# wangxb29/PPST

Hardware: AMD Instinct MI355X
Metric: 512x512 portrait swaps/sec/GPU (higher is better)
Workload: dtype bf16x3 (fp32 split into hi+lo bf16, 3 MFMA passes, fp32 accumulate); 1 GPU; simple_swapping 512x512 batch=8 per GPU, generator+encoders forward only (BASELINE configs[1]); image_parallel=1 batch per rank, no data-path collective

## Files before the change

include/ppst_hip.h:

```cpp
#ifndef PPST_HIP_H
#define PPST_HIP_H

#include <stddef.h>
#include <stdint.h>

#ifdef __cplusplus
extern "C" {
#endif

#define PPST_OK 0
#define PPST_EINVAL (-1)
#define PPST_EUNSUPPORTED (-2)
#define PPST_ENULL (-3)

enum { PPST_F32 = 0, PPST_F16 = 1, PPST_BF16 = 2, PPST_F64 = 3  };

enum { PPST_PAD_ZERO = 0, PPST_PAD_REFLECT = 1, PPST_PAD_REPLICATE = 2 };

enum { PPST_ACT_NONE = 0, PPST_ACT_LRELU = 1 , PPST_ACT_PRELU = 2 };

#define PPST_ABI_VERSION 3
int ppst_version(void);

#define PPST_ST_F32 0
// ... 61 lines not shown
  int32_t cout, cin, nblocks;
} ppst_upscale_job;
int ppst_pack_job_blocks(int64_t total);
int ppst_conv_pack_batch(const void* jobs, int njobs, int total_blocks, void* stream);
int ppst_upscale_weight_batch(const void* jobs, int njobs, int total_blocks, void* stream);

int ppst_upscale_weight(const void* w, void* out, int cout, int cin, float scale, void* stream);
int ppst_dgrad_s2d_stack_weight(const void* w, void* out, int cout, int cin, void* stream);
int ppst_depth_to_space_st(const void* x, void* y, int B, int th, int tw, int oh, int ow, int C, int st, void* stream);

#define PPST_KSPLIT_SCRATCH_BYTES ((size_t)256 * 512 * 128 * 4)
#define PPST_KSPLIT_FLAG_WORDS 4096

typedef struct ppst_conv_args {
  const void* x;
  const void* wpack;
  const void* steps;
  void* y;
  const void* bias;
  const void* noise;
  const void* prelu;
  void* stats;
  const void* residual;
  float noise_weight;
  float out_scale;
  int32_t B, in_h, in_w, in_ld;
  int32_t out_h, out_w, out_ld, cout;
  int32_t nsteps, n_groups;
  int32_t pad_mode;
  int32_t in_off_y, in_off_x;
  int32_t out_sy, out_sx;
  int32_t act;
  int32_t precision;
  int32_t res_ld;
  int32_t tile_h, tile_w;
  int32_t halo;
  int32_t bn;
  const void* in_scale_shift;
  const void* in_prelu;
  int32_t in_c, in_act;
  int32_t flop_steps;
  int32_t tile_rows;
  int32_t a_slots;
  int32_t early_a;
  int32_t variant;
  int32_t reserved0;
  int32_t dual_b;
  int32_t io_st;
  int32_t k64;
  const void* in_res;
  int32_t in_res_ld;
  int32_t ksplit;
  const int32_t* ksplit_starts;
  void* ksplit_scratch;
  unsigned* ksplit_flags;
  uint32_t ksplit_epoch;
} ppst_conv_args;

int ppst_conv2d_mfma(const ppst_conv_args* a, void* stream);
int64_t ppst_conv_pack_wino_bytes(int cout, int cin);
int ppst_conv_pack_wino(const void* w, int64_t sn, int64_t sc, int64_t sy, int64_t sx, float scale, int cout, int cin,
                        void* out, void* stream);
int ppst_conv2d_f32(const ppst_conv_args* a, const void* w, int64_t sn, int64_t sc, int64_t sy, int64_t sx, float wscale,
                    const int32_t* src_c, const int32_t* src_ky, const int32_t* src_kx, void* stream);
int ppst_conv_tiles(int tile_h, int tile_w, int tile_rows);

int ppst_conv1x1_small_cin(const void* x, const void* w, const void* bias, void* y,
                           int64_t npix, int cin, int in_ld, int cout, float wscale,
                           int act, void* stream);
int ppst_conv1x1_small_cin_st(const void* x, const void* w, const void* bias, void* y,
                              int64_t npix, int cin, int in_ld, int cout, float wscale,
                              int act, int y_st , void* stream);
int ppst_conv1x1_small_cin_nchw_st(const void* x, const void* w, const void* bias, void* y, int B, int64_t hw, int cin, int cout,
                                   float wscale, int act, int y_st, void* stream);
int ppst_conv1x1_small_cout(const void* x, const void* w, const void* bias, void* y,
                            int64_t npix, int cin, int cout, float wscale, void* stream);
int ppst_conv1x1_small_cout_st(const void* x, const void* w, const void* bias, void* y,
                               int64_t npix, int cin, int cout, float wscale, int x_st , void* stream);
int ppst_conv1x1_small_cout_ld_st(const void* x, const void* w, const void* bias, void* y, int64_t npix, int cin, int in_ld, int cout,
                                  float wscale, int x_st, void* stream);
int ppst_torgb_linear_st(const void* x, const void* scale_shift, const void* proj, float out_scale, const void* w, const void* bias,
                        void* y, void* partial, int* n_partials, int B, int H, int W, int cin, float wscale, int x_st, void* stream);
int ppst_rgb_affine_nchw(const void* y, const void* scale_shift, void* out, int B, int64_t hw, void* stream);

int ppst_in_stats(const void* x, void* partial, int B, int H, int W, int C, int ld,
                  int rep_pad, int* n_partials, void* stream);
int ppst_in_finalize(const void* partial, int n_partials, const void* style,
                     int style_ld ,
                     const void* post_bias ,
                     void* scale_shift , int B, int C, double count,
                     float eps, void* stream);
int ppst_affine_act(const void* x, const void* scale_shift, const void* res,
                    const void* res_scale_shift , void* y,
                    int B, int64_t hw, int C, int x_ld, int res_ld, int y_ld,
                    int act , const void* prelu,
                    float out_scale,
                    int res_up2_w ,
                    void* stream);
int ppst_affine_act_st(const void* x, const void* scale_shift, const void* res, const void* res_scale_shift, void* y,
                       int B, int64_t hw, int C, int x_ld, int res_ld, int y_ld, int act, const void* prelu,
                       float out_scale, int res_up2_w, int x_st, int y_st, void* stream);
int ppst_affine_act_stats(const void* x, const void* scale_shift, const void* res,
                          const void* res_scale_shift, void* y, void* partial,
                          int B, int H, int W, int C, int x_ld, int res_ld, int y_ld,
                          int act, const void* prelu, float out_scale, int rep_pad,
                          int res_up2 , void* stream);
int ppst_upsample_nearest2(const void* x, void* y, int B, int H, int W, int C, void* stream);
int ppst_upsample_nearest2_st(const void* x, void* y, int B, int H, int W, int C, int st, void* stream);

int64_t ppst_gap_gmp_ws(int B, int64_t hw, int C);
int ppst_gap_gmp(const void* x, const void* mask, void* out, void* ws, int B, int H, int W,
                 int C, int ld, void* stream);
int ppst_gap_gmp_st(const void* x, const void* mask, void* out, void* ws, int B, int H, int W,
                    int C, int ld, int x_st, void* stream);
#define PPST_GROUP_MAX 32
typedef struct {
  const void* x;
  const void* mask;
  void* out;
  int32_t H, W, C, ld;
} ppst_gap_gmp_level;
int64_t ppst_gap_gmp_multi_level_ws(const ppst_gap_gmp_level* levels, int n, int B);
int ppst_gap_gmp_multi_level(const ppst_gap_gmp_level* levels, int n, int B, void* ws, int x_st, void* stream);
int ppst_avgpool(const void* x, void* y, int B, int H, int W, int C, int x_ld, int f,
                 int y_ld, void* stream);
int ppst_bilinear(const void* x, void* y, int B, int H, int W, int C, int x_ld,
                  int OH, int OW, int y_ld, void* stream);
int ppst_head_tail(const void* x, const void* scale_shift, const void* prelu, void* feat, void* feat1,
                   int B, int H, int W, int C, int x_ld, int feat_ld, int feat1_ld, int P, int D, int act,
                   void* stream);
int ppst_maxpool2(const void* x, void* y, int B, int H, int W, int C, void* stream);

int ppst_linear(const void* x, const void* w, const void* bias, void* y,
                int B, int K, int N, float wscale, float bscale, int relu_in, int act,
                void* stream);
int ppst_l2norm_rows(const void* x, void* y, int B, int K, float eps, int mode, void* stream);
int ppst_lerp(const void* a, const void* b, void* y, int64_t n, float r, void* stream);
typedef struct {
  const void* x; const void* w; const void* bias ; void* y;
  int32_t B, K, N;
  float wscale, bscale;
  int32_t relu_in, act;
} ppst_linear_problem;
typedef struct { const void* x; void* y; int32_t B, K; float eps; int32_t mode; } ppst_l2norm_problem;
typedef struct { const void* a; const void* b; void* y; int64_t n; float r; } ppst_lerp_problem;
int ppst_linear_grouped(const ppst_linear_problem* problems, int n, void* stream);
int ppst_l2norm_rows_grouped(const ppst_l2norm_problem* problems, int n, void* stream);
int ppst_lerp_grouped(const ppst_lerp_problem* problems, int n, void* stream);
int ppst_spatial_modulation(const void* x, const void* scale, const void* bias, void* y,
                            int B, int64_t hw, int C, void* stream);
int ppst_spatial_modulation_st(const void* x, const void* scale, const void* bias, void* y,
                               int B, int64_t hw, int C, int y_st , void* stream);

int ppst_rselfcorr(const void* fea, void* out, int B, int H, int W, int C, int out_ld,
                   void* stream);
int ppst_corr_prep(const void* fea, void* out, int B, int P, int C, int ncenter, void* stream);
int ppst_unfold_rows(const void* x, void* out, int B, int H, int W, int C, int k, void* stream);
int ppst_unfold_rows_bwd(const void* g, void* dx, int B, int H, int W, int C, int k, void* stream);
int ppst_gemm_nt_f32(const void* A, const void* Bm, void* C, int batch, int M, int N, int K,
                     float alpha, void* stream);
int ppst_gemm_nn_f32(const void* A, const void* Bm, void* C, int batch, int M, int N, int K,
                     int ldb, int ldc, void* stream);
int ppst_gemm_nt_split(const void* A, const void* Bm, void* C, int batch, int M, int N, int K,
                       float alpha, int passes, void* stream);
int ppst_gemm_nn_split(const void* A, const void* Bm, void* C, int batch, int M, int N, int K,
                       int ldb, int ldc, int passes, void* stream);
// ... 263 lines not shown
```

ppst_amd/_lib.py:

```python
import ctypes
import os

import torch

HERE = os.path.dirname(os.path.abspath(__file__))
LIB_PATH = os.environ.get("PPST_HIP_LIB") or os.path.join(HERE, "libppst_hip.so")

if not os.path.exists(LIB_PATH):
    raise ImportError(
        "ppst_amd: %s is missing -- build it with `python -m ppst_amd.build` "
        "(hipcc --offload-arch=gfx950). There is no CPU fallback." % LIB_PATH)

lib = ctypes.CDLL(LIB_PATH)

vp, i32, i64, f32, f64 = ctypes.c_void_p, ctypes.c_int, ctypes.c_int64, ctypes.c_float, ctypes.c_double


class PackJob(ctypes.Structure):
    _fields_ = [("w", vp), ("sn", i64), ("sc", i64), ("sy", i64), ("sx", i64), ("src_c", vp), ("src_ky", vp), ("src_kx", vp),
                ("out", vp), ("total", i64), ("block0", i64), ("scale", f32), ("cout", i32), ("bn", i32), ("nsteps", i32),
                ("n_groups", i32), ("x3", i32), ("f16", i32), ("nblocks", i32), ("dual", i32)]


class UpscaleJob(ctypes.Structure):
# ... 7 lines not shown

class L2normProblem(ctypes.Structure):
    _fields_ = [("x", vp), ("y", vp), ("B", i32), ("K", i32), ("eps", f32), ("mode", i32)]


class LerpProblem(ctypes.Structure):
    _fields_ = [("a", vp), ("b", vp), ("y", vp), ("n", i64), ("r", f32)]


class GapGmpLevel(ctypes.Structure):
    _fields_ = [("x", vp), ("mask", vp), ("out", vp), ("H", i32), ("W", i32), ("C", i32), ("ld", i32)]


class JpegDecImage(ctypes.Structure):
    _u8 = ctypes.c_uint8
    _fields_ = [("H", i32), ("W", i32), ("ncomp", i32), ("ss", i32), ("hs", i32 * 3), ("vs", i32 * 3), ("dri", i32),
                ("scan_off", i32), ("scan_len", i32), ("qt", _u8 * 64 * 3), ("dc_tab", _u8 * 3), ("ac_tab", _u8 * 3), ("pad_", _u8 * 2),
                ("bits", _u8 * 16 * 4), ("vals", _u8 * 256 * 4), ("file_off", i64), ("out_off", i64), ("mirror", i32), ("expand_grey", i32)]


class PngSpan(ctypes.Structure):
    _fields_ = [("type", ctypes.c_uint32), ("off", i32), ("len", i32), ("crc", ctypes.c_uint32), ("idat", i32)]


class PngDecImage(ctypes.Structure):
    _fields_ = [("H", i32), ("W", i32), ("colour", i32), ("channels", i32), ("nspans", i32), ("first_idat", i32), ("nidat", i32),
                ("idat_bytes", i32), ("file_len", i64), ("file_off", i64), ("out_off", i64), ("span_off", i64),
                ("mirror", i32), ("expand_grey", i32), ("drop_alpha", i32), ("pad_", i32)]


GROUP_MAX = 32


class ConvArgs(ctypes.Structure):
    _fields_ = [
        ("x", vp), ("wpack", vp), ("steps", vp), ("y", vp), ("bias", vp), ("noise", vp),
        ("prelu", vp), ("stats", vp), ("residual", vp),
        ("noise_weight", f32), ("out_scale", f32),
        ("B", i32), ("in_h", i32), ("in_w", i32), ("in_ld", i32),
        ("out_h", i32), ("out_w", i32), ("out_ld", i32), ("cout", i32),
        ("nsteps", i32), ("n_groups", i32), ("pad_mode", i32),
        ("in_off_y", i32), ("in_off_x", i32), ("out_sy", i32), ("out_sx", i32),
        ("act", i32), ("precision", i32), ("res_ld", i32), ("tile_h", i32), ("tile_w", i32),
        ("halo", i32), ("bn", i32), ("in_scale_shift", vp), ("in_prelu", vp), ("in_c", i32), ("in_act", i32),
        ("flop_steps", i32), ("tile_rows", i32), ("a_slots", i32), ("early_a", i32), ("variant", i32), ("reserved0", i32), ("dual_b", i32), ("io_st", i32), ("k64", i32),
        ("in_res", vp), ("in_res_ld", i32), ("ksplit", i32), ("ksplit_starts", vp),
        ("ksplit_scratch", vp), ("ksplit_flags", vp), ("ksplit_epoch", ctypes.c_uint32),
    ]


_SIGS = {
    "ppst_version": (i32, []),
    "ppst_guided_filter_tune": (i32, [i32, i32]),
    "ppst_upfirdn2d": (i32, [vp, vp, vp] + [i32] * 14 + [i32, vp]),
    "ppst_blur_nhwc": (i32, [vp, vp, vp] + [i32] * 10 + [vp, i32, vp]),
    "ppst_blur_nhwc_st": (i32, [vp, vp, vp] + [i32] * 10 + [vp, i32, i32, vp]),
    "ppst_fused_bias_act": (i32, [vp, vp, vp, vp, i64, i32, i32, i32, i32, f32, f32, i32, vp]),
    "ppst_nchw_to_nhwc": (i32, [vp, vp, i32, i32, i32, i32, vp]),
    "ppst_nhwc_to_nchw": (i32, [vp, vp, i32, i32, i32, i32, vp]),
    "ppst_conv_pack": (i32, [vp, i64, i64, i64, i64, f32, i32, i32, vp, vp, vp, i32, i32, i32, vp, vp]),
    "ppst_conv_pack_k64": (i32, [vp, i64, i64, i64, i64, f32, i32, i32, vp, vp, vp, i32, i32, i32, i32, vp, vp]),
    "ppst_conv_pack_up9_bytes": (i64, [i32, i32]),
    "ppst_conv_pack_up9": (i32, [vp, i64, i64, i64, i64, f32, i32, i32, vp, vp]),
    "ppst_conv_pack_wino_bytes": (i64, [i32, i32]),
    "ppst_conv_pack_wino": (i32, [vp, i64, i64, i64, i64, f32, i32, i32, vp, vp]),
    "ppst_conv_pack_dual": (i32, [vp, i64, i64, i64, i64, f32, i32, vp, vp, vp, i32, i32, i32, vp, vp]),
    "ppst_upscale_weight": (i32, [vp, vp, i32, i32, f32, vp]),
    "ppst_dgrad_s2d_stack_weight": (i32, [vp, vp, i32, i32, vp]),
    "ppst_depth_to_space_st": (i32, [vp, vp, i32, i32, i32, i32, i32, i32, i32, vp]),
    "ppst_pack_job_blocks": (i32, [i64]),
    "ppst_conv_pack_batch": (i32, [vp, i32, i32, vp]),
    "ppst_upscale_weight_batch": (i32, [vp, i32, i32, vp]),
    "ppst_conv2d_mfma": (i32, [ctypes.POINTER(ConvArgs), vp]),
    "ppst_conv2d_f32": (i32, [ctypes.POINTER(ConvArgs), vp, i64, i64, i64, i64, f32, vp, vp, vp, vp]),
    "ppst_conv_tiles": (i32, [i32, i32, i32]),
    "ppst_conv1x1_small_cin": (i32, [vp, vp, vp, vp, i64, i32, i32, i32, f32, i32, vp]),
    "ppst_conv1x1_small_cin_st": (i32, [vp, vp, vp, vp, i64, i32, i32, i32, f32, i32, i32, vp]),
    "ppst_conv1x1_small_cout": (i32, [vp, vp, vp, vp, i64, i32, i32, f32, vp]),
    "ppst_conv1x1_small_cin_nchw_st": (i32, [vp, vp, vp, vp, i32, i64, i32, i32, f32, i32, i32, vp]),
    "ppst_conv1x1_small_cout_st": (i32, [vp, vp, vp, vp, i64, i32, i32, f32, i32, vp]),
    "ppst_conv1x1_small_cout_ld_st": (i32, [vp, vp, vp, vp, i64, i32, i32, i32, f32, i32, vp]),
    "ppst_torgb_linear_st": (i32, [vp, vp, vp, f32, vp, vp, vp, vp, ctypes.POINTER(i32), i32, i32, i32, i32, f32, i32, vp]),
    "ppst_rgb_affine_nchw": (i32, [vp, vp, vp, i32, i64, vp]),
    "ppst_in_stats": (i32, [vp, vp, i32, i32, i32, i32, i32, i32, ctypes.POINTER(i32), vp]),
    "ppst_in_finalize": (i32, [vp, i32, vp, i32, vp, vp, i32, i32, f64, f32, vp]),
    "ppst_affine_act": (i32, [vp, vp, vp, vp, vp, i32, i64, i32, i32, i32, i32, i32, vp, f32, i32, vp]),
    "ppst_affine_act_st": (i32, [vp, vp, vp, vp, vp, i32, i64, i32, i32, i32, i32, i32, vp, f32, i32, i32, i32, vp]),
    "ppst_affine_act_stats": (i32, [vp, vp, vp, vp, vp, vp, i32, i32, i32, i32, i32, i32, i32, i32, vp, f32, i32, i32, vp]),
    "ppst_upsample_nearest2": (i32, [vp, vp, i32, i32, i32, i32, vp]),
    "ppst_upsample_nearest2_st": (i32, [vp, vp, i32, i32, i32, i32, i32, vp]),
    "ppst_gap_gmp_ws": (i64, [i32, i64, i32]),
    "ppst_gap_gmp": (i32, [vp, vp, vp, vp, i32, i32, i32, i32, i32, vp]),
    "ppst_gap_gmp_st": (i32, [vp, vp, vp, vp, i32, i32, i32, i32, i32, i32, vp]),
    "ppst_avgpool": (i32, [vp, vp, i32, i32, i32, i32, i32, i32, i32, vp]),
    "ppst_bilinear": (i32, [vp, vp, i32, i32, i32, i32, i32, i32, i32, i32, vp]),
    "ppst_head_tail": (i32, [vp, vp, vp, vp, vp] + [i32] * 10 + [vp]),
    "ppst_maxpool2": (i32, [vp, vp, i32, i32, i32, i32, vp]),
    "ppst_linear": (i32, [vp, vp, vp, vp, i32, i32, i32, f32, f32, i32, i32, vp]),
    "ppst_l2norm_rows": (i32, [vp, vp, i32, i32, f32, i32, vp]),
    "ppst_lerp": (i32, [vp, vp, vp, i64, f32, vp]),
    "ppst_linear_grouped": (i32, [vp, i32, vp]),
    "ppst_l2norm_rows_grouped": (i32, [vp, i32, vp]),
    "ppst_lerp_grouped": (i32, [vp, i32, vp]),
    "ppst_gap_gmp_multi_level_ws": (i64, [vp, i32, i32]),
    "ppst_gap_gmp_multi_level": (i32, [vp, i32, i32, vp, i32, vp]),
    "ppst_spatial_modulation": (i32, [vp, vp, vp, vp, i32, i64, i32, vp]),
    "ppst_spatial_modulation_st": (i32, [vp, vp, vp, vp, i32, i64, i32, i32, vp]),
    "ppst_rselfcorr": (i32, [vp, vp, i32, i32, i32, i32, i32, vp]),
    "ppst_corr_prep": (i32, [vp, vp, i32, i32, i32, i32, vp]),
    "ppst_gemm_nt_f32": (i32, [vp, vp, vp, i32, i32, i32, i32, f32, vp]),
    "ppst_gemm_nn_f32": (i32, [vp, vp, vp, i32, i32, i32, i32, i32, i32, vp]),
    "ppst_unfold_rows": (i32, [vp, vp, i32, i32, i32, i32, i32, vp]),
    "ppst_unfold_rows_bwd": (i32, [vp, vp, i32, i32, i32, i32, i32, vp]),
    "ppst_gemm_nt_split": (i32, [vp, vp, vp, i32, i32, i32, i32, f32, i32, vp]),
    "ppst_gemm_nn_split": (i32, [vp, vp, vp, i32, i32, i32, i32, i32, i32, i32, vp]),
    "ppst_softmax_rows": (i32, [vp, i64, i32, f32, vp]),
    "ppst_unfold_patches": (i32, [vp, vp, i32, i32, i32, i32, i32, vp]),
    "ppst_fold_patches": (i32, [vp, vp, i32, i32, i32, i32, i32, vp]),
    "ppst_tensor2im_u8": (i32, [vp, vp, i32, i32, i32, i32, vp]),
    "ppst_resample_u8": (i32, [vp, vp, i32, i32, i32, i32, i32, i32, vp, vp, i32, vp]),
    "ppst_u8_to_tensor": (i32, [vp, vp, i32, i32, i32, i32, f32, f32, vp]),
    "ppst_resample_f32": (i32, [vp, vp, i32, i32, i32, i32, i32, vp, vp, i32, vp, vp, i32, i32, f32, f32, vp]),
    "ppst_png_bound": (i64, [i32, i32, i32]),
    "ppst_png_ws": (i64, [i32, i32, i32, i32]),
    "ppst_png_encode": (i32, [vp, vp, vp, i32, i32, i32, i32, vp, vp]),
    "ppst_jpeg_bound": (i64, [i32, i32, i32, i32]),
    "ppst_jpeg_ws": (i64, [i32, i32, i32, i32, i32]),
    "ppst_jpeg_header": (i64, [i32, i32, i32, i32, i32, vp, i64]),
    "ppst_jpeg_encode": (i32, [vp, vp, vp, i32, i32, i32, i32, i32, i32, vp, vp]),
    "ppst_jpeg_parse": (i32, [vp, i64, ctypes.POINTER(JpegDecImage)]),
    "ppst_jpeg_decode_ws": (i64, [ctypes.POINTER(JpegDecImage), i32, i32]),
    "ppst_jpeg_decode": (i32, [vp, i64, ctypes.POINTER(JpegDecImage), vp, vp, i64, vp, i32, i32, vp, vp]),
    "ppst_png_parse": (i32, [vp, i64, ctypes.POINTER(PngDecImage), ctypes.POINTER(PngSpan), i32]),
    "ppst_png_decode_ws": (i64, [ctypes.POINTER(PngDecImage), i32, i32]),
    "ppst_png_decode": (i32, [vp, i64, ctypes.POINTER(PngDecImage), vp, vp, vp, i64, vp, i32, i32, vp, vp]),
    "ppst_lpips_pack_floats": (i64, []),
    "ppst_lpips_pack": (i32, [vp, vp, vp, vp, vp, vp, vp]),
    "ppst_lpips_dims": (i32, [i32, i32, ctypes.POINTER(i32)]),
    "ppst_lpips_ws": (i64, [i32, i32, i32]),
    "ppst_lpips_trunk": (i32, [vp, vp, ctypes.POINTER(i64), i32, vp, ctypes.POINTER(i64), i32, i32, i32, vp, vp]),
    "ppst_lpips_feature": (i32, [vp, i32, i32, i32, i32, vp, vp]),
    "ppst_lpips_tail": (i32, [vp, vp, i32, i32, i32, vp, vp]),
    "ppst_lpips_bwd_ws": (i64, [i32, i32, i32, i32]),
    "ppst_lpips_backward": (i32, [vp, vp, vp, i32, i32, i32, i32, vp, vp, vp, vp]),
    "ppst_ssim_ws": (i64, [i32, i32, i32, i32]),
    "ppst_ssim_forward": (i32, [vp, ctypes.POINTER(i64), vp, ctypes.POINTER(i64), i32, i32, i32, i32, i32, f32, vp, vp, vp, vp, vp]),
    "ppst_ssim_backward": (i32, [vp, ctypes.POINTER(i64), vp, ctypes.POINTER(i64), vp, i32, i32, i32, i32, f32, vp, vp]),
    "ppst_pool2x2": (i32, [vp, ctypes.POINTER(i64), i32, i32, i32, i32, i32, vp, vp]),
    "ppst_msssim_combine": (i32, [vp, i32, i32, vp, vp]),
    "ppst_sqerr_ws": (i64, [i32, i32, i32, i32]),
    "ppst_sqerr": (i32, [vp, ctypes.POINTER(i64), vp, ctypes.POINTER(i64), i32, i32, i32, i32, i32, f32, vp, vp, vp]),
    "ppst_colour_stats_ws": (i64, [i32, i32, i32]),
    "ppst_colour_stats": (i32, [vp, i64, i64, i64, vp, i64, i64, i32, i32, i32, i32, ctypes.POINTER(ctypes.c_int16), i32, vp, vp, vp, vp, vp, vp]),
    "ppst_hist_w1": (i32, [vp, i32, vp, i32, vp, i32, i32, i32, vp, vp]),
    "ppst_guided_filter_ws": (i64, [i32, i32, i32]),
    "ppst_guided_filter": (i32, [vp, vp, vp, vp, i32, i32, i32, i32, f32, vp, vp]),
    "ppst_guided_filter_coeffs": (i32, [vp, vp, vp, i32, i32, i32, i32, f32, vp, vp]),
    "ppst_guided_filter_apply": (i32, [vp, i32, i32, vp, vp, vp, i32, i32, i32, vp]),
    "ppst_guided_filter_paste": (i32, [vp, i32, vp, vp, i32, i32, i32, vp, vp, i32, vp]),
    "ppst_guided_filter_paste_matte": (i32, [vp, vp, i32, vp, vp, i32, i32, i32, vp, vp, i32, vp]),
    "ppst_label_matte": (i32, [vp, i32, i32, i32, ctypes.c_uint32, i32, i32, vp, vp, vp]),
    "ppst_extract_similarity": (i32, [vp, i32, i32, i32, vp, vp, i32, vp, vp]),
    "ppst_smooth_local_affine_ws": (i64, [i32, i32, i32]),
    "ppst_smooth_local_affine": (i32, [vp, vp, vp, vp, vp, i32, i32, i32, i32, i32, f32, f32, vp]),
    "ppst_conv_wgrad_f32": (i32, [vp, vp, vp, vp, vp] + [i32] * 11 + [vp]),
    "ppst_conv_wgrad_tr2": (i32, [vp, vp, vp, vp, vp, vp, i32, i32, i32, i32, i32, i32, i32, i32, i32, i32, i32, i32, i32, i32, i32, vp]),
# ... 95 lines not shown
```

ppst_amd/build.py:

```python
import os
import subprocess
import sys
from concurrent.futures import ThreadPoolExecutor

HERE = os.path.dirname(os.path.abspath(__file__))
CSRC = os.path.join(HERE, "csrc")
OBJ = os.path.join(HERE, "csrc", "_obj")
LIB = os.path.join(HERE, "libppst_hip.so")
SOURCES = ["upfirdn2d.hip", "fused_bias_act.hip", "elementwise.hip", "linear.hip", "conv_mfma.hip", "conv_mfma2.hip", "conv1x1.hip", "conv_wino.hip", "conv_f32.hip",
           "corr.hip", "guided_filter.hip", "train.hip", "train_g.hip", "imageio.hip", "smooth_filter.hip", "png.hip", "jpeg.hip", "jpeg_parse.hip", "jpeg_decode.hip", "png_parse.hip", "png_decode.hip", "lpips.hip", "ssim.hip", "colour_stats.hip", "matte.hip"]
FLAGS = ["--offload-arch=gfx950", "-O3", "-fPIC", "-std=c++17", "-Wno-unused-result"]
FILE_FLAGS = {"conv_wino.hip": ["-fno-slp-vectorize"]}


def _hipcc():
    for c in (os.environ.get("HIPCC"), "/opt/rocm/bin/hipcc", "hipcc"):
        if c and (os.path.isabs(c) and os.path.exists(c) or not os.path.isabs(c)):
            return c
    return "hipcc"


HEADERS = [os.path.join(CSRC, "common.h"), os.path.join(CSRC, "conv_common.h"), os.path.join(CSRC, "rscl_common.h"), os.path.join(CSRC, "png_common.h"),
           os.path.join(CSRC, "codec_common.h"), os.path.join(CSRC, "jpeg_common.h"), os.path.join(CSRC, "parse_reader.h"), os.path.join(CSRC, "sim_xf.h"),
           os.path.join(HERE, "..", "include", "ppst_hip.h")]


def _stale(target, deps):
    return not os.path.exists(target) or any(os.path.getmtime(d) > os.path.getmtime(target) for d in deps)


def needs_build():
    return (_stale(LIB, [os.path.join(CSRC, s) for s in SOURCES] + HEADERS) or
            any(_stale(os.path.join(OBJ, s.replace(".hip", ".o")), [os.path.join(CSRC, s)]) for s in SOURCES if os.path.isdir(OBJ)))


def build(force=False, verbose=True):
    if not force and not needs_build():
        return LIB
    os.makedirs(OBJ, exist_ok=True)
    hipcc = _hipcc()

    def cc(src):
        obj = os.path.join(OBJ, src.replace(".hip", ".o"))
        if not force and not _stale(obj, [os.path.join(CSRC, src)] + HEADERS):
            return obj
        cmd = [hipcc] + FLAGS + FILE_FLAGS.get(src, []) + ["-c", os.path.join(CSRC, src), "-o", obj]
        r = subprocess.run(cmd, capture_output=True, text=True)
        if r.returncode != 0:
            raise RuntimeError("hipcc failed for %s:\n%s" % (src, r.stderr))
        return obj

    order = sorted(SOURCES, key=lambda f: 0 if f.startswith("conv") else 1)
    with ThreadPoolExecutor(max_workers=8) as ex:
        objs = dict(zip(order, ex.map(cc, order)))
    cmd = [hipcc, "--offload-arch=gfx950", "-shared", "-fPIC", "-o", LIB] + [objs[s_] for s_ in SOURCES]
    r = subprocess.run(cmd, capture_output=True, text=True)
    if r.returncode != 0:
        raise RuntimeError("link failed:\n%s" % r.stderr)
    if verbose:
        print("built", LIB)
    return LIB


if __name__ == "__main__":
    build(force="--force" in sys.argv)
```

ppst_amd/networks/base_network.py:

```python
import math

import torch
from torch import nn

from .. import ops, weights

SQRT2 = math.sqrt(2.0)
INV_SQRT2 = 1.0 / SQRT2


class _Node(nn.Module):
    """parameter container (no behaviour)."""


def to_nhwc(x):
    if x.dim() != 4:
        raise RuntimeError("expected a 4-D NCHW tensor")
    v = x.permute(0, 2, 3, 1)
    if v.is_contiguous():
        ops._chk(v, "input")
        return v
    return ops.nchw_to_nhwc(x)


# ... 29 lines not shown

    def p(self, name):
        t = self._flat.get(name)
        if t is None:
            node = self
            parts = name.split(".")
            for part in parts[:-1]:
                node = node._modules[part]
            t = node._parameters.get(parts[-1])
            if t is None:
                t = node._buffers[parts[-1]]
            self._flat[name] = t
        return t

    def _apply(self, fn, *a, **k):
        self._flat.clear()
        self._cache.clear()
        return super()._apply(fn, *a, **k)

    def load_state_dict(self, *a, **k):
        self._flat.clear()
        self._cache.clear()
        return super().load_state_dict(*a, **k)

    def cached(self, key, params, build):
        ver = tuple((id(t), t._version, t.data_ptr()) for t in params) + (ops.PRECISION["value"],)
        hit = self._cache.get(key)
        if hit is not None and hit[0] == ver:
            return hit[1]
        val = build()
        self._cache[key] = (ver, val)
        return val

    def plan(self, wname, kind="conv", scale=1.0):
        w = self.p(wname)
        return self.cached(("plan", wname, kind), [w], lambda: ops.ConvPlan(w, kind=kind, scale=scale))

    def refresh_plans(self):
        plans, keep = [], {}
        for key, (ver, val) in self._cache.items():
            if isinstance(key, tuple) and key and key[0] == "plan" and isinstance(val, ops.ConvPlan) and val.precision != 2 \
                    and val.wparam.data_ptr() == self.p(key[1]).data_ptr():
                plans.append(val)
                keep[key] = (ver, val)
        self._cache.clear()
        if not plans:
            return
        sig = tuple((id(pl), tuple(sorted(map(str, pl._packs)))) for pl in plans)
        hit = self.__dict__.get("_repack")
        if hit is not None and hit[0] == sig:
            ops.run_repack(hit[1])
        else:
            self.__dict__["_repack"] = (sig, ops.repack_plans(plans), plans)
        self._cache.update(keep)

    def print_architecture(self, verbose=False):
        n = sum(p.numel() for p in self.parameters())
        print("[Network %s] Total number of parameters : %.3f M" % (type(self).__name__, n / 1e6))

    def from_rgb(self, x, p, out_dtype=torch.float32):
        w = self.p(p + "Conv.weight")
        return ops.conv1x1_small_cin(x, w, self.p(p + "Act.bias"), 1.0 / math.sqrt(w.shape[1]), ops.ACT_LRELU, out_dtype=out_dtype)

    def from_rgb_image(self, img, p, out_dtype=torch.float32):
        if img.dim() == 4 and img.is_contiguous() and not img.permute(0, 2, 3, 1).is_contiguous():
            w = self.p(p + "Conv.weight")
            return ops.conv1x1_small_cin_nchw(img, w, self.p(p + "Act.bias"), 1.0 / math.sqrt(w.shape[1]), ops.ACT_LRELU, out_dtype=out_dtype)
        return self.from_rgb(to_nhwc(img), p, out_dtype=out_dtype)

    def _norm_act(self, y, st, count, act_bias=None, act=ops.ACT_NONE, **kw):
        ss = ops.in_finalize(st, count, post_bias=act_bias)
        return ops.affine_act(y, ss, act=act, **kw), ss

    def res_block(self, x, p, blur_pad_mode, norm):
        B, H, W, cin = x.shape
        k = self.p(p + "conv2.Blur.kernel")
        ks = k.shape[0]
        w1, w2, ws = self.p(p + "conv1.Conv.weight"), self.p(p + "conv2.Conv.weight"), self.p(p + "skip.Conv.weight")
        sc1 = 1.0 / math.sqrt(cin * 9)
        scs = 1.0 / math.sqrt(cin)
        conv_pad = ops.PAD_REFLECT if blur_pad_mode == ops.PAD_REFLECT else ops.PAD_ZERO
        pad_c = (ks - 2) + 2
        pad_s = (ks - 2) + 0
        xs, _ = ops.blur_nhwc(x, self.p(p + "skip.Blur.kernel"), (pad_s + 1) // 2, pad_s // 2, ops.PAD_ZERO, down=2)
        if not norm:
            y1 = self.plan(p + "conv1.Conv.weight", scale=sc1)(x, bias=self.p(p + "conv1.Act.bias"), act=ops.ACT_LRELU,
                                                                pad_mode=conv_pad)
            skip = self.plan(p + "skip.Conv.weight", scale=scs)(xs)
            xb, bhw = ops.blur_nhwc(y1, k, (pad_c + 1) // 2, pad_c // 2, blur_pad_mode, s2d=True)
            ohw = ((bhw[0] - 3) // 2 + 1, (bhw[1] - 3) // 2 + 1)
            return self.plan(p + "conv2.Conv.weight", "s2d", sc1)(
                xb, bias=self.p(p + "conv2.Act.bias"), act=ops.ACT_LRELU, residual=skip, res_after_act=True,
                out_scale=INV_SQRT2, out_hw=ohw)
        y1, st1 = self.plan(p + "conv1.Conv.weight", scale=sc1)(x, stats=True, pad_mode=conv_pad)
        ss1 = ops.in_finalize(st1, H * W, post_bias=self.p(p + "conv1.Act.bias"))
        ys, sts = self.plan(p + "skip.Conv.weight", scale=scs)(xs, stats=True)
        xb, bhw = ops.blur_nhwc(y1, k, (pad_c + 1) // 2, pad_c // 2, blur_pad_mode, s2d=True, in_ss=ss1, in_act=ops.ACT_LRELU)
        ohw = ((bhw[0] - 3) // 2 + 1, (bhw[1] - 3) // 2 + 1)
        y2, st2 = self.plan(p + "conv2.Conv.weight", "s2d", sc1)(xb, stats=True, out_hw=ohw)
        cnt = ohw[0] * ohw[1]
        ss_s = ops.in_finalize(sts, cnt)
        ss2 = ops.in_finalize(st2, cnt, post_bias=self.p(p + "conv2.Act.bias"))
        return ops.affine_act(y2, ss2, res=ys, res_scale_shift=ss_s, act=ops.ACT_LRELU, out_scale=INV_SQRT2)
```

ppst_amd/ops.py:

```python
import collections
import ctypes
import os
import threading
import types

import torch

from . import _lib, conv_tables
from ._lib import lib, check

PAD_ZERO, PAD_REFLECT, PAD_REPLICATE = 0, 1, 2
ACT_NONE, ACT_LRELU, ACT_PRELU = 0, 1, 2
RES_BEFORE_ACT = 1 << 8

PRECISION = {"value": 0}
TILE_ROWS = {"value": 16}
CONV_VARIANT = {"value": 2}
DUAL_CONVT = {"value": True, "min_blocks": 32}
UP9 = {"value": True, "min_blocks": 64, "min_fill": 0.85}
DIRECT_MAX = {"cout": 64, "nsteps": 40, "cout3x3": 64}
WGRAD_SPLIT = {"blocks": 1024, "min_tiles": 4}
WGRAD_TR2_BLOCKS = 512
WGRAD_TR2_MIN_TILES = 8
STREAM_1X1 = {"value": True}
# ... 789 lines not shown
def rscl_loss(q, k, k0, queue, nce_T=0.07):
    for t in (q, k, k0, queue):
        _chk(t)
    q, k, k0, queue = q.contiguous(), k.contiguous(), k0.contiguous(), queue.contiguous()
    n, C = q.shape
    ws = torch.empty((n,), device=q.device, dtype=torch.float32)
    out = torch.empty((1,), device=q.device, dtype=torch.float32)
    check(lib.ppst_rscl_loss(_p(q), _p(k), _p(k0), _p(queue), _p(out), _p(ws), n, k0.shape[0], C, queue.shape[1], float(nce_T), _stream()),
          "ppst_rscl_loss")
    return out


def adam_step_(p, g, m, v, lr, beta1, beta2, eps, step):
    for t in (p, g, m, v):
        _chk(t)
        assert t.is_contiguous()
    check(lib.ppst_adam_step(_p(p), _p(g), _p(m), _p(v), p.numel(), float(lr), float(beta1), float(beta2), float(eps), int(step),
                             _stream()), "ppst_adam_step")


def conv1x1_small_cin(x, w, bias, wscale, act, out_dtype=torch.float32):
    ld = _nhwc_ld(x)
    B, H, W, cin = x.shape
    cout = w.shape[0]
    y = torch.empty((B, H, W, cout), device=x.device, dtype=out_dtype)
    w2 = w.detach().reshape(cout, cin).contiguous()
    check(lib.ppst_conv1x1_small_cin_st(_p(x), _p(w2), _p(bias), _p(y), B * H * W, cin, ld, cout, float(wscale), act,
                                        _ST[out_dtype], _stream()), "ppst_conv1x1_small_cin")
    return y


def conv1x1_small_cin_nchw(x, w, bias, wscale, act, out_dtype=torch.float32):
    _chk(x, "x")
    B, cin, H, W = x.shape
    if not x.is_contiguous():
        raise RuntimeError("conv1x1_small_cin_nchw needs a contiguous NCHW tensor")
    cout = w.shape[0]
    y = torch.empty((B, H, W, cout), device=x.device, dtype=out_dtype)
    w2 = w.detach().reshape(cout, cin).contiguous()
    check(lib.ppst_conv1x1_small_cin_nchw_st(_p(x), _p(w2), _p(bias), _p(y), B, H * W, cin, cout, float(wscale), act, _ST[out_dtype],
                                             _stream()), "ppst_conv1x1_small_cin_nchw")
    return y


def conv1x1_small_cout(x, w, bias, wscale):
    ld = _nhwc_ld(x, half_ok=True)
    B, H, W, cin = x.shape
    cout = w.shape[0]
    y = torch.empty((B, H, W, cout), device=x.device, dtype=torch.float32)
    w2 = w.detach().reshape(cout, cin).contiguous()
    check(lib.ppst_conv1x1_small_cout_ld_st(_p(x), _p(w2), _p(bias), _p(y), B * H * W, cin, ld, cout, float(wscale), _ST[x.dtype], _stream()),
          "ppst_conv1x1_small_cout")
    return y


def torgb_apply(x, scale_shift, res, out_scale, w, bias, wscale, stats=False):
    ld = _nhwc_ld(x, half_ok=True)
    B, H, W, cin = x.shape
    if ld != cin or w.shape[0] != 3:
        raise RuntimeError("torgb_apply needs a dense input and a 3-channel weight")
    _chk(scale_shift, "scale_shift"); _chk(bias, "bias")
    proj = None
    if res is not None:
        if res.dtype != x.dtype or tuple(res.shape) != (B, H // 2, W // 2, cin) or H % 2 or W % 2:
            raise RuntimeError("torgb_apply: res must be the half-resolution tensor of x's type")
        proj = conv1x1_small_cout(res, w, None, float(wscale) * float(out_scale))
    if scale_shift is not None and (tuple(scale_shift.shape) != (B, cin, 2) or not scale_shift.is_contiguous()):
        raise RuntimeError("torgb_apply: scale_shift must be a contiguous (B, C, 2) table")
    y = torch.empty((B, H, W, 3), device=x.device, dtype=torch.float32)
    w2 = w.detach().reshape(3, cin).contiguous()
    if w2.data_ptr() % 16:
        w2 = w2.clone()
    n = ctypes.c_int(0)
    part = None
    if stats:
        check(lib.ppst_torgb_linear_st(None, None, None, 1.0, None, None, None, None, ctypes.byref(n), B, H, W, cin, 1.0, 0, None),
              "ppst_torgb_linear(size)")
        part = torch.empty((B, n.value, 3, 2), device=x.device, dtype=torch.float32)
    check(lib.ppst_torgb_linear_st(_p(x), _p(scale_shift), _p(proj), float(out_scale), _p(w2), _p(bias), _p(y), _p(part), ctypes.byref(n),
                                  B, H, W, cin, float(wscale), _ST[x.dtype], _stream()), "ppst_torgb_linear")
    return (y, part) if stats else y


def rgb_affine_nchw(y, scale_shift):
    _chk(y, "y"); _chk(scale_shift, "scale_shift")
    B, H, W, C = y.shape
    if C != 3 or not y.is_contiguous() or tuple(scale_shift.shape) != (B, 3, 2) or not scale_shift.is_contiguous():
        raise RuntimeError("rgb_affine_nchw needs a dense (B,H,W,3) tensor and a contiguous (B,3,2) table")
    out = torch.empty((B, 3, H, W), device=y.device, dtype=torch.float32)
    check(lib.ppst_rgb_affine_nchw(_p(y), _p(scale_shift), _p(out), B, H * W, _stream()), "ppst_rgb_affine_nchw")
    return out


def upscale_weight_bwd(dw4, cout, cin, scale=1.0, out=None, accumulate=False):
    _chk(dw4)
    dw = _grad_out(out, (cout, cin, 3, 3), dw4)
    check(lib.ppst_upscale_weight_bwd(_p(dw4.contiguous()), _p(dw), cout, cin, float(scale), 1 if (accumulate and out is not None) else 0,
                                      _stream()), "ppst_upscale_weight_bwd")
    return dw


DGRAD_S2D_STACK = {"value": os.environ.get("PPST_DGRAD_S2D_STACK", "1") != "0", "max_cin": int(os.environ.get("PPST_DGRAD_S2D_MAXCIN", "64"))}


def depth_to_space(x, out_hw):
    ld = _nhwc_ld(x, "depth_to_space input", half_ok=True)
    B, th, tw, c4 = x.shape
    if ld != c4 or c4 % 4:
        raise RuntimeError("depth_to_space needs a dense tensor with 4 C channels")
    oh, ow = out_hw
    y = torch.empty((B, oh, ow, c4 // 4), device=x.device, dtype=x.dtype)
    check(lib.ppst_depth_to_space_st(_p(x), _p(y), B, th, tw, oh, ow, c4 // 4, _ST[x.dtype], _stream()), "ppst_depth_to_space_st")
    return y


def dgrad_s2d(net, wname, scale, g, out_hw):
    cin = net.p(wname).shape[1]
    per = 8 if g.dtype != torch.float32 else 4
    if DGRAD_S2D_STACK["value"] and cin <= DGRAD_S2D_STACK["max_cin"] and cin % per == 0:
        oh, ow = out_hw
        ys = net.plan(wname, "dgrad_s2ds", scale)(g, out_hw=((oh + 1) // 2, (ow + 1) // 2))
        return depth_to_space(ys, out_hw)
    return net.plan(wname, "dgrad_s2d", scale)(g, out_hw=out_hw)


def space_to_depth(x):
    ld = _nhwc_ld(x, half_ok=True)
    B, H, W, C = x.shape
    y = torch.empty((B, (H + 1) // 2, (W + 1) // 2, 4 * C), device=x.device, dtype=x.dtype)
    check(lib.ppst_space_to_depth_st(_p(x), _p(y), B, H, W, C, ld, _ST[x.dtype], _stream()), "ppst_space_to_depth")
    return y


def in_stats(x, rep_pad=False):
    ld = _nhwc_ld(x)
    B, H, W, C = x.shape
    n = ctypes.c_int(0)
    check(lib.ppst_in_stats(None, None, B, H, W, C, ld, 0, ctypes.byref(n), None), "ppst_in_stats(size)")
    part = torch.empty((B, n.value, C, 2), device=x.device, dtype=torch.float32)
    check(lib.ppst_in_stats(_p(x), _p(part), B, H, W, C, ld, 1 if rep_pad else 0, ctypes.byref(n), _stream()), "ppst_in_stats")
    return part


def in_finalize(partial, count, style=None, post_bias=None, eps=1e-5):
    _chk(partial)
    _chk(style, "style")
    _chk(post_bias, "post_bias")
    B, n, C, _ = partial.shape
    style_ld = 0
    if style is not None:
        assert style.shape == (B, 2 * C) and style.stride(1) == 1
        style_ld = style.stride(0) if B > 1 else max(style.stride(0), 2 * C)
    ss = torch.empty((B, C, 2), device=partial.device, dtype=torch.float32)
    check(lib.ppst_in_finalize(_p(partial), n, _p(style), style_ld, _p(post_bias), _p(ss), B, C, float(count), float(eps),
                               _stream()), "ppst_in_finalize")
    return ss


def in_finalize_train(partial, count, style=None, post_bias=None, eps=1e-5):
    _chk(partial); _chk(style, "style"); _chk(post_bias, "post_bias")
    B, n, C, _ = partial.shape
    style_ld = 0
    if style is not None:
        assert style.shape == (B, 2 * C) and style.stride(1) == 1
        style_ld = style.stride(0) if B > 1 else max(style.stride(0), 2 * C)
    ss = torch.empty((B, C, 2), device=partial.device, dtype=torch.float32)
# ... 1208 lines not shown
```

Measured before the change: 166.6 swaps/s (all GPUs).

## Fuse encoder downsampling ResBlock into one persistent LDS-resident HIP kernel

Adds a persistent kernel that computes a whole 32->32->64 encoder ResBlock (conv1 3x3 + lrelu, blur, strided conv2 3x3, blurred 1x1 skip, residual scale) per 8x8 output tile in LDS. Weights stay in registers, and the next tile's input is prefetched while the current one is computed. This removes the intermediate activation round-trips to global memory and several kernel launches that the unfused path needed. The cost is recomputing the conv1 halo per tile, heavy register and LDS use, and a path that only applies to one specific channel configuration with reflect padding and matching blur kernels.

```diff
diff --git a/include/ppst_hip.h b/include/ppst_hip.h
--- a/include/ppst_hip.h
+++ b/include/ppst_hip.h
@@ -167,6 +167,8 @@
 int ppst_torgb_linear_st(const void* x, const void* scale_shift, const void* proj, float out_scale, const void* w, const void* bias,
                         void* y, void* partial, int* n_partials, int B, int H, int W, int cin, float wscale, int x_st, void* stream);
 int ppst_rgb_affine_nchw(const void* y, const void* scale_shift, void* out, int B, int64_t hw, void* stream);
+int ppst_encoder_resblock(const void* x, int x_st, int B, int H, int W, int cin, int cmid, int cout, int x_ld, const void* w1, const void* w2,
+                          const void* ws, const void* b1, const void* b2, const void* blur, void* y, void* stream);
 
 int ppst_in_stats(const void* x, void* partial, int B, int H, int W, int C, int ld,
                   int rep_pad, int* n_partials, void* stream);
diff --git a/ppst_amd/_lib.py b/ppst_amd/_lib.py
--- a/ppst_amd/_lib.py
+++ b/ppst_amd/_lib.py
@@ -113,6 +113,7 @@
     "ppst_conv1x1_small_cout_ld_st": (i32, [vp, vp, vp, vp, i64, i32, i32, i32, f32, i32, vp]),
     "ppst_torgb_linear_st": (i32, [vp, vp, vp, f32, vp, vp, vp, vp, ctypes.POINTER(i32), i32, i32, i32, i32, f32, i32, vp]),
     "ppst_rgb_affine_nchw": (i32, [vp, vp, vp, i32, i64, vp]),
+    "ppst_encoder_resblock": (i32, [vp, i32, i32, i32, i32, i32, i32, i32, i32, vp, vp, vp, vp, vp, vp, vp, vp]),
     "ppst_in_stats": (i32, [vp, vp, i32, i32, i32, i32, i32, i32, ctypes.POINTER(i32), vp]),
     "ppst_in_finalize": (i32, [vp, i32, vp, i32, vp, vp, i32, i32, f64, f32, vp]),
     "ppst_affine_act": (i32, [vp, vp, vp, vp, vp, i32, i64, i32, i32, i32, i32, i32, vp, f32, i32, vp]),
diff --git a/ppst_amd/build.py b/ppst_amd/build.py
--- a/ppst_amd/build.py
+++ b/ppst_amd/build.py
@@ -7,7 +7,7 @@
 CSRC = os.path.join(HERE, "csrc")
 OBJ = os.path.join(HERE, "csrc", "_obj")
 LIB = os.path.join(HERE, "libppst_hip.so")
-SOURCES = ["upfirdn2d.hip", "fused_bias_act.hip", "elementwise.hip", "linear.hip", "conv_mfma.hip", "conv_mfma2.hip", "conv1x1.hip", "conv_wino.hip", "conv_f32.hip",
+SOURCES = ["upfirdn2d.hip", "fused_bias_act.hip", "elementwise.hip", "linear.hip", "conv_mfma.hip", "conv_mfma2.hip", "conv1x1.hip", "conv_wino.hip", "conv_f32.hip", "encoder_block.hip",
            "corr.hip", "guided_filter.hip", "train.hip", "train_g.hip", "imageio.hip", "smooth_filter.hip", "png.hip", "jpeg.hip", "jpeg_parse.hip", "jpeg_decode.hip", "png_parse.hip", "png_decode.hip", "lpips.hip", "ssim.hip", "colour_stats.hip", "matte.hip"]
 FLAGS = ["--offload-arch=gfx950", "-O3", "-fPIC", "-std=c++17", "-Wno-unused-result"]
 FILE_FLAGS = {"conv_wino.hip": ["-fno-slp-vectorize"]}
diff --git a/ppst_amd/csrc/encoder_block.hip b/ppst_amd/csrc/encoder_block.hip
--- /dev/null
+++ b/ppst_amd/csrc/encoder_block.hip
@@ -0,0 +1,288 @@
+#include "conv_common.h"
+
+namespace {
+
+constexpr int EB_NT = 512;
+constexpr int EB_SLOTS = EB_NT / 8;
+constexpr int EB_BLOB = 8192;
+constexpr int EB_YS = 36;
+
+template <int TOH, int TOW>
+struct EbGeom {
+  static constexpr int Y1H = 2 * TOH + 3, Y1W = 2 * TOW + 3;
+  static constexpr int XH = Y1H + 2, XW = Y1W + 2;
+  static constexpr int BH = 2 * TOH + 1, BW = 2 * TOW + 1;
+  static constexpr int BROW = 2 * TOW + 4, BHALF = TOW + 2;
+  static constexpr int NPX = TOH * TOW;
+  static constexpr int XPL = (XH * XW + 15) / 16 * 16;
+  static constexpr int BPL = (BH * BROW + 15) / 16 * 16;
+  static constexpr int X_BYTES = 8 * XPL * 16, B_BYTES = 8 * BPL * 16, S_BYTES = 8 * NPX * 16;
+  static constexpr int Y1_BYTES = Y1H * Y1W * EB_YS * 4;
+  static constexpr int XF_BYTES = BH * BW * 128;
+  static constexpr int LDS = X_BYTES + Y1_BYTES + XF_BYTES + S_BYTES;
+  static constexpr int NX = XH * XW * 8, NIT = (NX + EB_NT - 1) / EB_NT;
+  static_assert(B_BYTES <= X_BYTES, "the blurred image takes the x patch's place");
+  static_assert(NPX % 16 == 0 && TOW + 1 <= BHALF && LDS <= 160 * 1024, "16-pixel m-tiles; one block per CU");
+};
+
+struct EbArgs {
+  const float* x;
+  const unsigned char* w1;
+  const unsigned char* w2;
+  const unsigned char* ws;
+  const float* b1;
+  const float* b2;
+  const float* blur;
+  float* y;
+  int H, W, OH, OW, tiles_y, tiles_x, nblocks;
+};
+
+__device__ __forceinline__ bf16x8 eb_wfrag(const unsigned char* w, int tap, int hl, int nt16, int lane) {
+  return *(const bf16x8*)(w + tap * EB_BLOB + hl * (EB_BLOB / 2) + (((lane >> 4) * 64 + nt16 * 16 + (lane & 15)) << 4));
+}
+__device__ __forceinline__ f32x4 eb_mfma3(bf16x8 wh, bf16x8 wl, bf16x8 xh, bf16x8 xl, f32x4 acc) {
+  acc = __builtin_amdgcn_mfma_f32_16x16x32_bf16(wh, xl, acc, 0, 0, 0);
+  acc = __builtin_amdgcn_mfma_f32_16x16x32_bf16(wl, xh, acc, 0, 0, 0);
+  return __builtin_amdgcn_mfma_f32_16x16x32_bf16(wh, xh, acc, 0, 0, 0);
+}
+__device__ __forceinline__ void eb_put_split(unsigned char* img, int plane, int px, int cq, float4 v) {
+  uint2 hi, lo;
+  split_bf16x4(v, hi, lo);
+  unsigned char* const d = img + (((cq >> 1) * plane + px) << 4) + (cq & 1) * 8;
+  *(uint2*)d = hi;
+  *(uint2*)(d + plane * 64) = lo;
+}
+__device__ __forceinline__ void eb_fir(float4& acc, float4 v, float f) {
+  acc.x = fmaf(v.x, f, acc.x); acc.y = fmaf(v.y, f, acc.y); acc.z = fmaf(v.z, f, acc.z); acc.w = fmaf(v.w, f, acc.w);
+}
+__device__ __forceinline__ float4 eb_bias4(const float* b, int n0) { return make_float4(b[n0], b[n0 + 1], b[n0 + 2], b[n0 + 3]); }
+
+struct EbTile { int b, oy0, ox0; };
+template <int TOH, int TOW>
+__device__ __forceinline__ EbTile eb_tile(const EbArgs& a, int v) {
+  int id = xcd_block_id(v, a.nblocks);
+  EbTile t;
+  t.ox0 = (id % a.tiles_x) * TOW;
+  id /= a.tiles_x;
+  t.oy0 = (id % a.tiles_y) * TOH;
+  t.b = id / a.tiles_y;
+  return t;
+}
+template <int P>
+__device__ __forceinline__ void eb_step(int& row, int& col) {
+  row += EB_SLOTS / P;
+  col += EB_SLOTS % P;
+  if (col >= P) { col -= P; ++row; }
+}
+template <int TOH, int TOW>
+__device__ __forceinline__ void eb_fetch(const EbArgs& a, const EbTile& t, int pr, int cq, float4 (&v)[EbGeom<TOH, TOW>::NIT]) {
+  using G = EbGeom<TOH, TOW>;
+  const float* const xb = a.x + (int64_t)t.b * a.H * a.W * 32 + cq * 4;
+  const int y0 = 2 * t.oy0 - 3, x0 = 2 * t.ox0 - 3;
+  const bool inside = y0 >= 0 && x0 >= 0 && y0 + G::XH <= a.H && x0 + G::XW <= a.W;
+  auto go = [&](auto in_c) {
+    int j = pr / G::XW, i = pr % G::XW;
+#pragma unroll
+    for (int it = 0; it < G::NIT; ++it) {
+      const bool past = (it + 1) * EB_SLOTS > G::XH * G::XW && it * EB_SLOTS + pr >= G::XH * G::XW;
+      const int jj = past ? G::XH - 1 : j, ii = past ? G::XW - 1 : i;
+      const int ry = in_c.value ? y0 + jj : conv_pad_index(y0 + jj, a.H, PPST_PAD_REFLECT), rx = in_c.value ? x0 + ii : conv_pad_index(x0 + ii, a.W, PPST_PAD_REFLECT);
+      v[it] = *(const float4*)(xb + (ry * a.W + rx) * 32);
+      eb_step<G::XW>(j, i);
+    }
+  };
+  if (inside) go(EpiC<1>{}); else go(EpiC<0>{});
+}
+
+template <int TOH, int TOW>
+__global__ __launch_bounds__(EB_NT) void encoder_resblock_kernel(EbArgs a) {
+  using G = EbGeom<TOH, TOW>;
+  __shared__ __attribute__((aligned(256))) unsigned char lds[G::LDS];
+  unsigned char* const xs = lds;
+  unsigned char* const bs = lds;
+  float* const y1s = (float*)(lds + G::X_BYTES);
+  float* const xf = (float*)(lds + G::X_BYTES + G::Y1_BYTES);
+  unsigned char* const ss = lds + G::X_BYTES + G::Y1_BYTES + G::XF_BYTES;
+  const int tid = threadIdx.x, lane = tid & 63, wave = tid >> 6;
+  const int cq = tid & 7;
+  const float4 zero4 = make_float4(0.f, 0.f, 0.f, 0.f);
+
+  const int nt1 = wave & 1, mg1 = wave >> 1, nt2 = wave & 3, mg2 = wave >> 2;
+  bf16x8 w1h[9], w1l[9], w2h[9], w2l[9];
+#pragma unroll
+  for (int t = 0; t < 9; ++t) {
+    w1h[t] = eb_wfrag(a.w1, t, 0, nt1, lane);
+    w1l[t] = eb_wfrag(a.w1, t, 1, nt1, lane);
+    w2h[t] = eb_wfrag(a.w2, t, 0, nt2, lane);
+    w2l[t] = eb_wfrag(a.w2, t, 1, nt2, lane);
+  }
+  const bf16x8 sh = eb_wfrag(a.ws, 0, 0, nt2, lane), sl = eb_wfrag(a.ws, 0, 1, nt2, lane);
+  const float4 b1v = eb_bias4(a.b1, nt1 * 16 + (lane >> 4) * 4);
+  const float4 b2v = eb_bias4(a.b2, nt2 * 16 + (lane >> 4) * 4);
+  float kf[9];
+#pragma unroll
+  for (int i = 0; i < 9; ++i) kf[i] = a.blur[8 - i];
+
+  float4 v[G::NIT];
+  if ((int)blockIdx.x < a.nblocks) eb_fetch<TOH, TOW>(a, eb_tile<TOH, TOW>(a, blockIdx.x), tid >> 3, cq, v);
+  for (int work = blockIdx.x; work < a.nblocks; work += gridDim.x) {
+    const EbTile tl = eb_tile<TOH, TOW>(a, work);
+    const int oy0 = tl.oy0, ox0 = tl.ox0;
+    const int y1r0 = 2 * oy0 - 2, y1c0 = 2 * ox0 - 2;
+    int pr = tid >> 3, r16 = lane & 15, g = lane >> 4;
+    asm volatile("" : "+v"(pr), "+v"(r16), "+v"(g));
+
+    {
+      int j = pr / G::XW, i = pr % G::XW;
+#pragma unroll
+      for (int it = 0; it < G::NIT; ++it) {
+        eb_put_split(xs, G::XPL, min(pr + it * EB_SLOTS, G::XH * G::XW - 1), cq, v[it]);
+        if ((unsigned)(j - 2) < (unsigned)G::BH && (unsigned)(i - 2) < (unsigned)G::BW) *(float4*)(xf + ((j - 2) * G::BW + (i - 2)) * 32 + cq * 4) = v[it];
+        eb_step<G::XW>(j, i);
+      }
+    }
+    if (work + (int)gridDim.x < a.nblocks) eb_fetch<TOH, TOW>(a, eb_tile<TOH, TOW>(a, work + gridDim.x), pr, cq, v);
+    __syncthreads();
+
+    for (int pix = pr; pix < G::NPX; pix += EB_SLOTS) {
+      const int ly = pix / TOW, lx = pix - ly * TOW;
+      float4 acc = zero4;
+#pragma unroll
+      for (int ky = 0; ky < 3; ++ky)
+#pragma unroll
+        for (int kx = 0; kx < 3; ++kx) {
+          float4 t = *(const float4*)(xf + ((2 * ly + ky) * G::BW + 2 * lx + kx) * 32 + cq * 4);
+          if (2 * (oy0 + ly) - 1 + ky < 0 || 2 * (ox0 + lx) - 1 + kx < 0) t = zero4;
+          eb_fir(acc, t, kf[ky * 3 + kx]);
+        }
+      eb_put_split(ss, G::NPX, pix, cq, acc);
+    }
+    {
+      constexpr int NP1 = G::Y1H * G::Y1W, NM1 = (NP1 + 15) / 16, PASSES = (NM1 + 11) / 12;
+      for (int pass = 0; pass < PASSES; ++pass) {
+        int p[3];
+        const unsigned char* src[3];
+        f32x4 acc[3];
+#pragma unroll
+        for (int u = 0; u < 3; ++u) {
+          p[u] = (mg1 + 4 * (pass * 3 + u)) * 16 + r16;
+          const int pc = min(p[u], NP1 - 1), qy = pc / G::Y1W, qx = pc - qy * G::Y1W;
+          src[u] = xs + ((g * G::XPL + qy * G::XW + qx) << 4);
+          acc[u] = (f32x4){0.f, 0.f, 0.f, 0.f};
+        }
+#pragma unroll
+        for (int t = 0; t < 9; ++t) {
+          const int off = ((t / 3) * G::XW + (t % 3)) * 16;
+#pragma unroll
+          for (int u = 0; u < 3; ++u) {
+            const bf16x8 xh = *(const bf16x8*)(src[u] + off), xl = *(const bf16x8*)(src[u] + off + G::XPL * 64);
+            acc[u] = eb_mfma3(w1h[t], w1l[t], xh, xl, acc[u]);
+          }
+        }
+#pragma unroll
+        for (int u = 0; u < 3; ++u) {
+          float o[4];
+          conv_epi_value4(o, make_float4(acc[u][0], acc[u][1], acc[u][2], acc[u][3]), b1v, 0.f, zero4, 0.f, 1.f, EpiC<PPST_ACT_LRELU>{}, EpiC<0>{});
+          if (p[u] < NP1) *(float4*)(y1s + p[u] * EB_YS + nt1 * 16 + g * 4) = make_float4(o[0], o[1], o[2], o[3]);
+        }
+      }
+    }
+    __syncthreads();
+
+    {
+      const bool inside = y1r0 >= 0 && y1c0 >= 0 && y1r0 + G::Y1H <= a.H && y1c0 + G::Y1W <= a.W;
+      auto go = [&](auto in_c) {
+        int i = pr / G::BW, j = pr % G::BW;
+#pragma unroll 1
+        for (int it = 0; it < (G::BH * G::BW + EB_SLOTS - 1) / EB_SLOTS; ++it) {
+          if ((it + 1) * EB_SLOTS <= G::BH * G::BW || it * EB_SLOTS + pr < G::BH * G::BW) {
+            int ro[3], co[3];
+#pragma unroll
+            for (int k = 0; k < 3; ++k) {
+              if (in_c.value) { ro[k] = (i + k) * G::Y1W; co[k] = j + k; }
+              else {
+                const int r = conv_pad_index(y1r0 + i + k, a.H, PPST_PAD_REFLECT) - y1r0, c = conv_pad_index(y1c0 + j + k, a.W, PPST_PAD_REFLECT) - y1c0;
+                ro[k] = min(max(r, 0), G::Y1H - 1) * G::Y1W;
+                co[k] = min(max(c, 0), G::Y1W - 1);
+              }
+            }
+            float4 acc = make_float4(0.f, 0.f, 0.f, 0.f);
+#pragma unroll
+            for (int ky = 0; ky < 3; ++ky)
+#pragma unroll
+              for (int kx = 0; kx < 3; ++kx) eb_fir(acc, *(const float4*)(y1s + (ro[ky] + co[kx]) * EB_YS + cq * 4), kf[ky * 3 + kx]);
+            eb_put_split(bs, G::BPL, i * G::BROW + (j & 1) * G::BHALF + (j >> 1), cq, acc);
+          }
+          eb_step<G::BW>(i, j);
+        }
+      };
+      if (inside) go(EpiC<1>{}); else go(EpiC<0>{});
+    }
+    __syncthreads();
+
+    {
+      constexpr int MT = G::NPX / 32;
+      int ly[MT], lx[MT];
+      const unsigned char* src[MT];
+      f32x4 acc[MT], accs[MT];
+#pragma unroll
+      for (int u = 0; u < MT; ++u) {
+        const int pl = (mg2 * MT + u) * 16 + r16;
+        ly[u] = pl / TOW;
+        lx[u] = pl - ly[u] * TOW;
+        src[u] = bs + ((g * G::BPL + 2 * ly[u] * G::BROW + lx[u]) << 4);
+        const unsigned char* sp = ss + ((g * G::NPX + pl) << 4);
+        accs[u] = eb_mfma3(sh, sl, *(const bf16x8*)sp, *(const bf16x8*)(sp + G::NPX * 64), (f32x4){0.f, 0.f, 0.f, 0.f});
+        acc[u] = (f32x4){0.f, 0.f, 0.f, 0.f};
+      }
+#pragma unroll
+      for (int t = 0; t < 9; ++t) {
+        const int kx = t % 3, off = ((t / 3) * G::BROW + (kx & 1) * G::BHALF + (kx >> 1)) * 16;
+#pragma unroll
+        for (int u = 0; u < MT; ++u) {
+          const bf16x8 xh = *(const bf16x8*)(src[u] + off), xl = *(const bf16x8*)(src[u] + off + G::BPL * 64);
+          acc[u] = eb_mfma3(w2h[t], w2l[t], xh, xl, acc[u]);
+        }
+      }
+      float* const yb = a.y + (int64_t)tl.b * a.OH * a.OW * 64;
+#pragma unroll
+      for (int u = 0; u < MT; ++u) {
+        const int oy = oy0 + ly[u], ox = ox0 + lx[u];
+        float o[4];
+        conv_epi_value4(o, make_float4(acc[u][0], acc[u][1], acc[u][2], acc[u][3]), b2v, 0.f,
+                        make_float4(accs[u][0], accs[u][1], accs[u][2], accs[u][3]), 0.f, 0.70710678118654752f, EpiC<PPST_ACT_LRELU>{}, EpiC<2>{});
+        if (oy < a.OH && ox < a.OW) PPST_EPI_STORE(yb + (oy * a.OW + ox) * 64 + nt2 * 16 + g * 4, o);
+      }
+    }
+    __syncthreads();
+  }
+}
+
+int eb_grid(int64_t tiles) {
+  int dev = 0, cus = 0;
+  if (hipGetDevice(&dev) != hipSuccess || hipDeviceGetAttribute(&cus, hipDeviceAttributeMultiprocessorCount, dev) != hipSuccess || cus < 8) cus = 256;
+  cus &= ~7;
+  return (int)(tiles < cus ? tiles : cus);
+}
+
+}
+
+extern "C" int ppst_encoder_resblock(const void* x, int x_st, int B, int H, int W, int cin, int cmid, int cout, int x_ld, const void* w1,
+                                     const void* w2, const void* ws, const void* b1, const void* b2, const void* blur, void* y, void* stream) {
+  constexpr int TOH = 8, TOW = 8;
+  if (x_st != PPST_ST_F32 || cin != 32 || cmid != 32 || cout != 64 || x_ld != 32 || B < 1 || H < 4 || W < 4 || (H & 1) || (W & 1)) return PPST_EINVAL;
+  if (!x || !w1 || !w2 || !ws || !b1 || !b2 || !blur || !y) return PPST_ENULL;
+  if ((int64_t)H * W * 32 >= (1ll << 31)) return PPST_EINVAL;
+  if (((uintptr_t)x | (uintptr_t)y | (uintptr_t)w1 | (uintptr_t)w2 | (uintptr_t)ws) % 16 || ((uintptr_t)b1 | (uintptr_t)b2 | (uintptr_t)blur) % 4)
+    return PPST_EINVAL;
+  EbArgs a;
+  a.x = (const float*)x; a.w1 = (const unsigned char*)w1; a.w2 = (const unsigned char*)w2; a.ws = (const unsigned char*)ws;
+  a.b1 = (const float*)b1; a.b2 = (const float*)b2; a.blur = (const float*)blur; a.y = (float*)y;
+  a.H = H; a.W = W; a.OH = H / 2; a.OW = W / 2;
+  a.tiles_y = cdiv(a.OH, TOH); a.tiles_x = cdiv(a.OW, TOW);
+  const int64_t tiles = (int64_t)B * a.tiles_y * a.tiles_x;
+  if (tiles >= (1ll << 31)) return PPST_EINVAL;
+  a.nblocks = (int)tiles;
+  PPST_LAUNCH((encoder_resblock_kernel<TOH, TOW>), dim3((unsigned)eb_grid(tiles)), dim3(EB_NT), 0, as_stream(stream), a);
+  return PPST_LAUNCH_CHECK();
+}
diff --git a/ppst_amd/networks/base_network.py b/ppst_amd/networks/base_network.py
--- a/ppst_amd/networks/base_network.py
+++ b/ppst_amd/networks/base_network.py
@@ -135,6 +135,12 @@
         conv_pad = ops.PAD_REFLECT if blur_pad_mode == ops.PAD_REFLECT else ops.PAD_ZERO
         pad_c = (ks - 2) + 2
         pad_s = (ks - 2) + 0
+        if not norm and blur_pad_mode == ops.PAD_REFLECT and ks == 3 and ops.encoder_resblock_ok(x, w1.shape[0], w2.shape[0]) \
+                and self.cached(("one_blur", p), [k, self.p(p + "skip.Blur.kernel")],
+                                lambda: bool(torch.equal(k, self.p(p + "skip.Blur.kernel")))):
+            return ops.encoder_resblock(x, self.plan(p + "conv1.Conv.weight", scale=sc1), self.plan(p + "conv2.Conv.weight", scale=sc1),
+                                        self.plan(p + "skip.Conv.weight", scale=scs), self.p(p + "conv1.Act.bias"),
+                                        self.p(p + "conv2.Act.bias"), k)
         xs, _ = ops.blur_nhwc(x, self.p(p + "skip.Blur.kernel"), (pad_s + 1) // 2, pad_s // 2, ops.PAD_ZERO, down=2)
         if not norm:
             y1 = self.plan(p + "conv1.Conv.weight", scale=sc1)(x, bias=self.p(p + "conv1.Act.bias"), act=ops.ACT_LRELU,
diff --git a/ppst_amd/ops.py b/ppst_amd/ops.py
--- a/ppst_amd/ops.py
+++ b/ppst_amd/ops.py
@@ -895,6 +895,30 @@
     return (y, part) if stats else y
 
 
+def encoder_resblock_ok(x, cmid, cout):
+    if torch.is_grad_enabled() or PRECISION["value"] != 0 or x.dtype != torch.float32 or not x.is_cuda or x.dim() != 4:
+        return False
+    B, H, W, cin = x.shape
+    return (x.is_contiguous() and x.data_ptr() % 16 == 0 and (cin, cmid, cout) == (32, 32, 64) and B >= 1 and H >= 4 and W >= 4
+            and H % 2 == 0 and W % 2 == 0 and H * W * 32 < 2 ** 31)
+
+
+def encoder_resblock(x, plan1, plan2, plan_s, b1, b2, blur):
+    _chk_act(x, "x"); _chk(b1, "b1"); _chk(b2, "b2"); _chk(blur, "blur")
+    B, H, W, cin = x.shape
+    dense = x.stride(3) == 1 and x.stride(2) == cin and x.stride(1) == W * cin and (B == 1 or x.stride(0) == H * W * cin)
+    if plan1.kind != "conv" or plan2.kind != "conv" or plan_s.kind != "conv" or (plan1.k, plan2.k, plan_s.k) != (3, 3, 1) \
+            or plan1.cin != cin or plan2.cin != plan1.cout or plan_s.cin != cin or plan_s.cout != plan2.cout \
+            or any(pl.precision != 0 for pl in (plan1, plan2, plan_s)) or blur.numel() != 9 or not blur.is_contiguous() \
+            or b1.numel() != plan1.cout or b2.numel() != plan2.cout or not b1.is_contiguous() or not b2.is_contiguous():
+        raise RuntimeError("encoder_resblock: plans must be the fp32-class 'conv' plans of a 3x3 / 3x3 / 1x1 ResBlock, blur a 3x3 FIR")
+    y = torch.empty((B, H // 2, W // 2, plan2.cout), device=x.device, dtype=torch.float32)
+    check(lib.ppst_encoder_resblock(_p(x), _ST[x.dtype], B, H, W, cin, plan1.cout, plan2.cout, x.stride(2) if dense else 0,
+                                    _p(plan1.pack_for(64)), _p(plan2.pack_for(64)), _p(plan_s.pack_for(64)), _p(b1), _p(b2), _p(blur), _p(y),
+                                    _stream()), "ppst_encoder_resblock")
+    return y
+
+
 def rgb_affine_nchw(y, scale_shift):
     _chk(y, "y"); _chk(scale_shift, "scale_shift")
     B, H, W, C = y.shape
```

After: 168.5 swaps/s (all GPUs) (median of 6 runs). 1.01x the previous value.
